# michelbarbeau/gr-uwspr

Hardware: NVIDIA B200
Metric: WSPR windows/sec (coarse+fine sync+demod) (higher is better)
Workload: dtype f32

## Files before the change

gr-uwspr_b200/csrc/capi.cu:

```cuda
#include <limits.h>
#include <math.h>
#include <stdio.h>
#include <stdlib.h>
#include <string.h>

#include <algorithm>
#include <chrono>
#include <future>
#include <string>
#include <thread>
#include <vector>

#include "common.cuh"
#include "../host/wspr_tables.h"

#ifndef M_PI
#define M_PI 3.14159265358979323846
#endif

namespace {

const int kMaxChunks = 1024;
const int kCounterSets = 15;
const int kCounterInts = 4 + 4 * kCounterSets;
// ... 1012 lines not shown
        for (int r = 0; r < d.n_rows; r++) memcpy(ps + (size_t)r * d.n_bins, &tmp[(size_t)r * d.nbp], sizeof(float) * d.n_bins);
    }
    if (psavg) CU(cudaMemcpy(psavg, ctx->b.psavg + slot * d.nbp, sizeof(float) * d.n_bins, cudaMemcpyDeviceToHost));
    return UWSPR_B200_OK;
}

int uwspr_b200_last_timing(const uwspr_b200_ctx *ctx, float ms[4])
{
    if (!ctx || !ms) return UWSPR_B200_E_PARAM;
    for (int q = 0; q < 4; q++) ms[q] = ctx->ms[q];
    return UWSPR_B200_OK;
}

int64_t uwspr_b200_launch_count(const uwspr_b200_ctx *ctx) { return ctx ? ctx->launches : 0; }

}
```

gr-uwspr_b200/csrc/common.cuh:

```cuda
#pragma once

#include <cuda_runtime.h>
#include <stdint.h>

#include "uwspr_b200.h"

#define UW_NSYM 162
#define UW_FFT_N 512
#define UW_HOP 128
#define UW_NK0 26
#define UW_NIFR 5
#define UW_NTRAJ 125
#define UW_SPS 256
#define UW_NP 45000
#define UW_MAX_TILE_W 40
#define UW_MAX_UNIQUE 192
#define UW_NQUAD 41

struct UwDims {
    int fl, n_rows, size, m, hpbm, finpb, noiseidx, maxfreqs, maxcand, maxdrift, cf;
    float df, min_snr, floor_val, threshold;
    int bin_lo, n_bins, nbp;
    int n_lin, n_hyp, n_unique;
    int off_min, off_max, tile_w;
// ... 77 lines not shown
                           const float *window, const float2 *twiddle, float *amp, float *ps_dbg,
                           float *psavg, UwPeak *peaks, int *npk, cudaStream_t s);
void uw_launch_worklist(const int *npk, int nwin, int cap, int *base, UwItem *items, int *counters,
                        int *set, cudaStream_t s);
void uw_launch_coarse(const UwDims &d, const float *amp, const UwPeak *peaks, const UwItem *items,
                      const int *total, int cap, const uint32_t *off4, const short *hyp_unique,
                      uwspr_b200_candidate_t *cands, int *ticket, int grid, cudaStream_t s);
struct UwFineWork {
    void *state;
    float4 *pbuf, *pE, *pbest, *tables;
    int *tickets;
    int slice;
};
cudaError_t uw_fine_work_alloc(UwFineWork *w, int slice);
void uw_fine_work_free(UwFineWork *w);
struct UwFineLaunch {
    int grid_points, grid_lags, grid_share;
    bool lag_share;
    bool reuse;
};
int uw_launch_fine(const UwDims &d, const float2 *x, const UwGeom &geom, const UwItem *items, const int *begin,
                   const int *end, int cap, const uwspr_b200_candidate_t *cands, int jig_first, int jig_count,
                   uwspr_b200_refined_t *refined, uwspr_b200_jiggle_t *jig, uint8_t *soft, int slice0,
                   const UwFineWork &w, const UwFineLaunch &l, cudaStream_t s);
int uw_coarse_fine_channels(uwspr_b200_ctx *ctx, const float *samples, int64_t win_stride, int wins_per_chan,
                            int64_t chan_stride, int nchan, int jig_first, int jig_count, int32_t *npk,
                            uwspr_b200_candidate_t *cands, int cap, int32_t *total);
int64_t uw_frontend_stream_launches(const uwspr_b200_frontend_stream *s);
size_t uw_coarse_smem_bytes(const UwDims &d);
int uw_coarse_setup(const UwDims &d);
int uw_fine_setup(int sm_count, bool lag_share, bool reuse, UwFineLaunch *l);
int uw_coarse_blocks_per_sm(const UwDims &d);
// ... 9 lines not shown
```

gr-uwspr_b200/csrc/fine.cu:

```cuda
#include "common.cuh"

#include <algorithm>
#include <cassert>

namespace {

constexpr int kThreads = 256;
constexpr int kWarps = kThreads / 32;
constexpr int kPB = 5;
constexpr int kKC1 = 8;
constexpr int kPitch1 = kKC1 + 2;
constexpr int kNChunk1 = UW_SPS / kKC1;
constexpr int kRows2 = 32;
constexpr int kPass2 = UW_NSYM / kRows2;
constexpr int kSpan2 = 128;
constexpr int kKCR = 32;
constexpr int kRing = kSpan2 + 2 * kKCR;
constexpr int kPitch2 = kRing + 1;
constexpr int kMaxJ = UWSPR_B200_NJIG;
constexpr int kLagPT = 5;
constexpr int kMemo = 24;
constexpr int kTickets = 16;
constexpr size_t kWarpSmem = 2 * 32 * kPitch1 * sizeof(float2) + 2 * 2 * kKC1 * 2 * sizeof(float4);
constexpr int kSlots1 = (kPB * UW_NSYM + 31) / 32;
constexpr int kSlotsRest = (kMaxJ * (UW_NSYM - kPass2 * kRows2) + 31) / 32;

struct FineCand {
    float f1, drift1, sync1;
    int shift1;
    int worth;
    int npt, nev;
    float pt_f0[kPB];
    int pt_lag[kPB];
    float pt_drift[kPB];
    float pt_ss[kPB];
    int ev[kPB];
    int tab[kPB];
    int ntab;
    float tab_f0[kPB], tab_drift[kPB];
    int memo_n;
    float memo_f0[kMemo], memo_drift[kMemo], memo_ss[kMemo];
    int memo_lag[kMemo];
    int nl;
    int e_lag[kMaxJ], e_jig[kMaxJ];
    float e_f0, e_drift;
    int best_have, best_lag, best_col;
    float best_f0, best_drift;
    int e_reuse;
    int xoff;
};

struct FineConst {
// ... 5 lines not shown
struct FineArgs {
    UwDims d;
    FineConst fc;
    const float2 *x;
    UwGeom geom;
    const UwItem *items;
    const uwspr_b200_candidate_t *cands;
    const int *begin_ptr, *end_ptr;
    int cap, slice0, slice_n;
    FineCand *st;
    float4 *pbuf;
    float4 *pE;
    float4 *pbest;
    float4 *tables;
    int *tickets;
    int jig_first, jig_count;
    int reuse;
    uwspr_b200_refined_t *refined;
    uwspr_b200_jiggle_t *jig;
    uint8_t *soft;
};

__device__ __forceinline__ int slice_count(const FineArgs &a)
{
    const int begin = *a.begin_ptr + a.slice0, end = min(*a.end_ptr, a.cap);
    return max(0, min(a.slice_n, end - begin));
}

__device__ __forceinline__ void cp_async_commit() { asm volatile("cp.async.commit_group;\n" ::: "memory"); }
template <int IMM> __device__ __forceinline__ void cp_async8_s(unsigned sdst, const void *gsrc, int bytes)
// ... 18 lines not shown
    double r = __ddiv_rn(__dmul_rn((double)(-sign), num), den);
    r = __ddiv_rn(__dmul_rn(r, (double)cf), 1500.0);
    return (float)r;
}

__device__ __forceinline__ uwspr_b200_candidate_t load_cand(const uwspr_b200_candidate_t *cands, int g)
{
    uwspr_b200_candidate_t cand = cands[g];
    if (cand.m_type != 0) {
        unsigned long long v1 = (unsigned long long)__double_as_longlong(cand.m_nonlinear.V1);
        cand.m_nonlinear.V1 = __longlong_as_double((long long)(v1 & 0xffffffff00000000ull));
    }
    return cand;
}

__device__ __forceinline__ float symbol_freq(const UwDims &d, const uwspr_b200_candidate_t &cand, float f0,
                                             float drift, int i)
{
    if (cand.m_type == 0) {
        const double a = __dmul_rn((double)drift, 0.5);
        const double b = __dsub_rn((double)(float)i, 81.0);
        return (float)__dadd_rn((double)f0, __ddiv_rn(__dmul_rn(a, b), 81.0));
    }
    const float t = d.nonlinear_intended_t ? (float)(i * 111 / 162) : 0.0f;
    return __fadd_rn(f0, slm_frequency_drift(cand.m_nonlinear.V1, cand.m_nonlinear.V2, cand.m_nonlinear.p1,
                                             cand.m_nonlinear.p2, (float)d.cf, t));
}

__device__ __forceinline__ void tone_seed(const FineConst &fc, float fp, int j, float &cd, float &sd)
{
    const double arg = __dmul_rn(fc.twopidt, (double)__fadd_rn(fp, fc.delta[j]));
    double sn, cs;
    sincos(arg, &sn, &cs);
    cd = (float)cs;
    sd = (float)sn;
}

#define UW_MAC2(inp, quad, xv, c, s)                                                             \
// ... 201 lines not shown
    extern __shared__ __align__(16) unsigned char smem_raw[];
    const int lane = threadIdx.x & 31, warp = threadIdx.x >> 5;
    WarpTile xt = reinterpret_cast<WarpTile>(smem_raw + (size_t)warp * kWarpSmem);
    TableTile tt = reinterpret_cast<TableTile>(smem_raw + (size_t)warp * kWarpSmem + 2 * 32 * kPitch1 * sizeof(float2));
    const int n = slice_count(a);
    const int begin = *a.begin_ptr + a.slice0;
    constexpr int kSlots = REST ? kSlotsRest : kSlots1;
    constexpr int s_lo = REST ? kPass2 * kRows2 : 0, s_cnt = REST ? UW_NSYM - kPass2 * kRows2 : UW_NSYM;
    for (;;) {
        int slot = 0;
        if (lane == 0) slot = atomicAdd(a.tickets + tk, 1);
        slot = __shfl_sync(0xffffffffu, slot, 0);
        if (slot >= n * kSlots) break;
        const int cidx = slot / kSlots, local = slot - cidx * kSlots;
        const FineCand &st = a.st[cidx];
        const int np = REST ? (st.worth == 1 ? st.nl : 0) : (lag_share && st.nev > 0 && st.tab[0] < 0) ? 0 : st.nev;
        const int ntask = np * s_cnt;
        if (local * 32 >= ntask) continue;
        const int g = begin + cidx;
        const uwspr_b200_candidate_t cand = load_cand(a.cands, g);
        const float2 *xw = a.x + st.xoff;
        const int task = local * 32 + lane;
        const bool live = task < ntask;
        const int tq = min(task, ntask - 1);
        const int q = tq / s_cnt;
        const int i = s_lo + (tq - q * s_cnt);
        float f0, drift;
        int lag, tab = -1;
        float4 *out;
        if (REST) {
            f0 = st.e_f0;
            drift = st.e_drift;
            lag = st.e_lag[q];
            out = a.pE + ((size_t)cidx * UW_NSYM + i) * kMaxJ + q;
        } else {
            const int pq = st.ev[q];
            f0 = st.pt_f0[pq];
            drift = st.pt_drift[pq];
            lag = st.pt_lag[pq];
            tab = st.tab[q];
            out = a.pbuf + ((size_t)cidx * UW_NSYM + i) * kPB + q;
        }
        if (!REST && __all_sync(0xffffffffu, tab >= 0)) {
            const int tab_a = __shfl_sync(0xffffffffu, tab, 0), tab_b = __shfl_sync(0xffffffffu, tab, 31);
            const float4 *tbase = a.tables + (size_t)cidx * kPB * (UW_SPS * 2);
            r1_task<true>(xt, tt, a.d, a.fc, xw, cand, live, f0, drift, lag, i, tbase + (size_t)tab_a * (UW_SPS * 2),
                          tbase + (size_t)tab_b * (UW_SPS * 2), tab == tab_a ? 0 : 1, out);
        } else {
            r1_task<false>(xt, tt, a.d, a.fc, xw, cand, live, f0, drift, lag, i, nullptr, nullptr, 0, out);
        }
    }
}

static_assert(UW_SPS % kKCR == 0 && kRing % 8 == 0, "chunks and lag offsets (multiples of 8) never straddle the wrap");

template <int IMM> __device__ __forceinline__ float2 lds_f2(unsigned addr)
// ... 329 lines not shown
        if (!RING || nl == kPB)
            lagshare_run<RING, kPB>(wsm, a.x, rp, rb, pe, cd, sd, inp, quad, nz);
        else
            lagshare_run<RING, kPB - 1>(wsm, a.x, rp, rb, pe, cd, sd, inp, quad, nz);
        if (live) {
            float4 *out = a.pbuf + ((size_t)cidx * UW_NSYM + i) * kPB;
#pragma unroll
            for (int e = 0; e < kPB; e++)
                if (e < nev)
                    out[e] = make_float4(tone_mag(uw_lo(inp[e][0]), uw_lo(quad[e][0])), tone_mag(uw_hi(inp[e][0]), uw_hi(quad[e][0])),
                                         tone_mag(uw_lo(inp[e][1]), uw_lo(quad[e][1])), tone_mag(uw_hi(inp[e][1]), uw_hi(quad[e][1])));
        }
    }
}

__device__ __forceinline__ bool const_freq(bool lin, bool intended_t, float drift)
{
    return lin ? (drift == 0.0f) : !intended_t;
}

__device__ __forceinline__ void stage_points(FineCand &st, int np, bool lin, bool intended_t)
{
    int nev = 0;
    for (int q = 0; q < np; q++) {
        int hit = -1;
        for (int m = 0; m < st.memo_n; m++)
            if (__float_as_uint(st.memo_f0[m]) == __float_as_uint(st.pt_f0[q]) && st.memo_lag[m] == st.pt_lag[q] &&
                __float_as_uint(st.memo_drift[m]) == __float_as_uint(st.pt_drift[q])) {
                hit = m;
                break;
            }
        if (hit >= 0)
            st.pt_ss[q] = st.memo_ss[hit];
        else
            st.ev[nev++] = q;
    }
// ... 5 lines not shown
        int t = -1;
        if (const_freq(lin, intended_t, st.pt_drift[q])) {
            for (int u = 0; u < ntab && t < 0; u++)
                if (__float_as_uint(st.tab_f0[u]) == __float_as_uint(st.pt_f0[q]) &&
                    __float_as_uint(st.tab_drift[u]) == __float_as_uint(st.pt_drift[q]))
                    t = u;
            if (t < 0) {
                t = ntab++;
                st.tab_f0[t] = st.pt_f0[q];
                st.tab_drift[t] = st.pt_drift[q];
            }
        }
        st.tab[e] = t;
    }
    st.ntab = ntab;
}

__device__ __forceinline__ void keep_point(FineCand &st, int q)
{
    st.best_col = -1;
    if (q < 0) return;
    for (int e = 0; e < st.nev; e++)
        if (st.ev[e] == q) {
            st.best_col = e;
            st.best_have = 1;
            st.best_f0 = st.pt_f0[q];
            st.best_lag = st.pt_lag[q];
            st.best_drift = st.pt_drift[q];
        }
}
// ... 10 lines not shown
    st.sync1 = syncmax;
    st.shift1 = (best >= 0) ? st.pt_lag[best] : 0;
    st.f1 = (best >= 0) ? st.pt_f0[best] : 0.0f;
    keep_point(st, best);
}

template <int STAGE>
__global__ void __launch_bounds__(256) k_fine_step(FineArgs a)
{
    const int n = slice_count(a);
    const int begin = *a.begin_ptr + a.slice0;
    const int gt = blockIdx.x * blockDim.x + threadIdx.x;
    const int cidx = gt >> 3, sub = gt & 7;
    const unsigned gmask = 0xffu << (threadIdx.x & 24);
    const bool have = cidx < n;
    __shared__ FineCand s_state[256 / 8];
    static_assert(sizeof(FineCand) % 4 == 0, "copied word by word");
    FineCand &gst = a.st[have ? cidx : 0];
    FineCand &st = s_state[threadIdx.x >> 3];
    if (have) {
        const int *src = reinterpret_cast<const int *>(&gst);
        int *dst = reinterpret_cast<int *>(&st);
        for (int k = sub; k < (int)(sizeof(FineCand) / 4); k += 8) dst[k] = STAGE >= 1 ? src[k] : 0;
    }
    __syncwarp(gmask);
    const int g = begin + cidx;
    const float minsync1 = 0.10f;
    const bool skip = have && STAGE >= 4 && st.worth != 1;
    if (STAGE >= 1 && have && !skip && sub < st.nev) {
        const float4 *p = a.pbuf + (size_t)cidx * UW_NSYM * kPB + sub;
        float ss = 0.0f, totp = 0.0f;
        constexpr int kBatch = 9;
        static_assert(UW_NSYM % kBatch == 0, "162 = 18 x 9");
        for (int i0 = 0; i0 < UW_NSYM; i0 += kBatch) {
            float4 vb[kBatch];
#pragma unroll
            for (int k = 0; k < kBatch; k++) vb[k] = p[(size_t)(i0 + k) * kPB];
#pragma unroll
            for (int k = 0; k < kBatch; k++) {
                const float4 v = vb[k];
                totp = __fadd_rn(__fadd_rn(__fadd_rn(__fadd_rn(totp, v.x), v.y), v.z), v.w);
                const float cmet = __fsub_rn(__fadd_rn(v.y, v.w), __fadd_rn(v.x, v.z));
                ss = uw_sync_bit(a.d.sync_words, i0 + k) ? __fadd_rn(ss, cmet) : __fsub_rn(ss, cmet);
// ... 6 lines not shown
    if (sub == 0) {
        const uwspr_b200_candidate_t cand = a.cands[g];
        const bool lin = cand.m_type == 0;
        if (STAGE == 0) {
            st.f1 = cand.freq;
            st.drift1 = lin ? cand.m_linear.drift : 0.0f;
            st.shift1 = cand.shift;
            st.sync1 = cand.sync;
            st.memo_n = 0;
            st.worth = -1;
            st.nl = 0;
            st.best_have = 0;
            st.best_col = -1;
            st.e_reuse = -1;
            st.xoff = (int)(uw_window_offset(a.geom, a.items[g].win) - uw_window_offset(a.geom, 0));
            if (cidx == 0)
                for (int q = 0; q < kTickets; q++) a.tickets[q] = 0;
        } else {
            for (int e = 0; e < st.nev && st.memo_n < kMemo; e++) {
                const int q = st.ev[e], m = st.memo_n++;
                st.memo_f0[m] = st.pt_f0[q];
                st.memo_lag[m] = st.pt_lag[q];
                st.memo_drift[m] = st.pt_drift[q];
                st.memo_ss[m] = st.pt_ss[q];
            }
        }
        if (STAGE == 1 || STAGE == 2 || STAGE == 4 || STAGE == 5) select_best(st);
        if (STAGE == 3) st.best_col = -1;
        if (STAGE == 3 && lin) {
            const float syncp = (st.pt_ss[0] > -1e30f) ? st.pt_ss[0] : -1e30f;
            const float syncm = (st.pt_ss[1] > -1e30f) ? st.pt_ss[1] : -1e30f;
            if (!(st.pt_ss[1] > -1e30f)) {
// ... 28 lines not shown
            const float fstep = STAGE == 1 ? 0.25f : 0.05f;
            for (int q = 0; q < 5; q++) {
                st.pt_f0[q] = __fadd_rn(f1, __fmul_rn((float)(q - 2), fstep));
                st.pt_lag[q] = shift1;
                st.pt_drift[q] = drift1;
            }
            np = 5;
        } else if (STAGE == 2 && lin) {
            for (int q = 0; q < 2; q++) {
                st.pt_f0[q] = __fadd_rn(f1, __fmul_rn(0.0f, 0.0f));
                st.pt_lag[q] = shift1;
                st.pt_drift[q] = (float)((double)drift1 + (q == 0 ? 0.5 : -0.5));
            }
            np = 2;
        }
        if (STAGE <= 4) stage_points(st, np, lin, a.d.nonlinear_intended_t != 0);
        const bool final_state = (STAGE == 3 && st.worth == 0) || STAGE == 5;
        if (final_state && a.refined) {
            uwspr_b200_refined_t r;
            r.f1 = st.f1;
            r.shift1 = st.shift1;
            r.drift1 = st.drift1;
            r.sync1 = st.sync1;
            r.worth_a_try = st.worth == 1 ? 1 : 0;
            r.reserved = 0;
            a.refined[g] = r;
        }
        if (STAGE == 5) {
            st.e_f0 = __fadd_rn(st.f1, __fmul_rn(0.0f, 0.0f));
            st.e_drift = st.drift1;
            const bool reuse = st.best_have && __float_as_uint(st.best_f0) == __float_as_uint(st.e_f0) &&
// ... 7 lines not shown
                if (idt >= a.jig_first && idt < a.jig_first + a.jig_count && !(reuse && idt == 0)) {
                    st.e_lag[nl] = st.shift1 + off;
                    st.e_jig[nl] = idt - a.jig_first;
                    nl++;
                }
            }
            st.nl = nl;
            st.nev = 0;
        }
    }
    __syncwarp(gmask);
    {
        const int *src = reinterpret_cast<const int *>(&st);
        int *dst = reinterpret_cast<int *>(&gst);
        for (int k = sub; k < (int)(sizeof(FineCand) / 4); k += 8) dst[k] = src[k];
    }
    if (STAGE >= 1 && st.best_col >= 0) {
        const float4 *src = a.pbuf + (size_t)cidx * UW_NSYM * kPB + st.best_col;
        float4 *dst = a.pbest + (size_t)cidx * UW_NSYM;
        for (int i = sub; i < UW_NSYM; i += 8) dst[i] = src[(size_t)i * kPB];
    }
    if (STAGE == 3 && st.worth == 0) {
        uint8_t *soft_g = a.soft ? a.soft + (long long)g * a.jig_count * UW_NSYM : nullptr;
        uwspr_b200_jiggle_t *jig_g = a.jig ? a.jig + (long long)g * a.jig_count : nullptr;
        if (soft_g)
            for (int t = sub; t < a.jig_count * UW_NSYM; t += 8) soft_g[t] = 0;
        if (jig_g)
            for (int t = sub; t < a.jig_count; t += 8) {
                uwspr_b200_jiggle_t z;
                z.sync = 0.0f;
// ... 72 lines not shown
    if (a.jig) {
        uwspr_b200_jiggle_t r;
        const float sy = (sync > -1e30f) ? sync : -1e30f;
        r.sync = sy;
        r.rms = (float)__dsqrt_rn(__ddiv_rn((double)(float)sq, 162.0));
        r.shift = kept ? st.shift1 : st.e_lag[slot];
        r.gate = (sy > minsync2 && r.rms > minrms) ? 1 : 0;
        a.jig[(long long)g * a.jig_count + jidx] = r;
    }
}

constexpr size_t kPointsSmem = (size_t)kWarps * kWarpSmem;

}

cudaError_t uw_fine_work_alloc(UwFineWork *w, int slice)
{
    *w = UwFineWork{};
    const size_t n = (size_t)slice;
    const size_t bytes[6] = { n * sizeof(FineCand), n * UW_NSYM * kPB * sizeof(float4), n * UW_NSYM * kMaxJ * sizeof(float4),
                              n * UW_NSYM * sizeof(float4), n * kPB * UW_SPS * 2 * sizeof(float4), kTickets * sizeof(int) };
    size_t at[7] = { 0 };
    for (int q = 0; q < 6; q++) at[q + 1] = at[q] + ((bytes[q] + 255) & ~(size_t)255);
    char *p = nullptr;
    const cudaError_t e = cudaMalloc(&p, at[6]);
    if (e != cudaSuccess) return e;
    *w = UwFineWork{ p, reinterpret_cast<float4 *>(p + at[1]), reinterpret_cast<float4 *>(p + at[2]),
                     reinterpret_cast<float4 *>(p + at[3]), reinterpret_cast<float4 *>(p + at[4]),
                     reinterpret_cast<int *>(p + at[5]), slice };
    return cudaMemset(w->tickets, 0, kTickets * sizeof(int));
}

void uw_fine_work_free(UwFineWork *w)
{
    if (w->state) cudaFree(w->state);
    *w = UwFineWork{};
}

int uw_fine_setup(int sm_count, bool lag_share, bool reuse, UwFineLaunch *l)
{
    if (cudaFuncSetAttribute(k_fine_lags, cudaFuncAttributeMaxDynamicSharedMemorySize, (int)sizeof(LagSmem)) != cudaSuccess) return 1;
    if (cudaFuncSetAttribute(k_fine_points<false>, cudaFuncAttributeMaxDynamicSharedMemorySize, (int)kPointsSmem) != cudaSuccess) return 1;
    if (cudaFuncSetAttribute(k_fine_points<true>, cudaFuncAttributeMaxDynamicSharedMemorySize, (int)kPointsSmem) != cudaSuccess) return 1;
    if (cudaFuncSetAttribute(k_fine_lagshare<false>, cudaFuncAttributeMaxDynamicSharedMemorySize, (int)kShareSmem) != cudaSuccess) return 1;
    if (cudaFuncSetAttribute(k_fine_lagshare<true>, cudaFuncAttributeMaxDynamicSharedMemorySize, (int)kShareSmem) != cudaSuccess) return 1;
    int n = 0, m = 0;
    const int points = (cudaOccupancyMaxActiveBlocksPerMultiprocessor(&n, k_fine_points<false>, kThreads, kPointsSmem) == cudaSuccess && n > 0) ? n : 1;
    const int lags = (cudaOccupancyMaxActiveBlocksPerMultiprocessor(&n, k_fine_lags, kThreads, sizeof(LagSmem)) == cudaSuccess && n > 0) ? n : 1;
    const bool ok = cudaOccupancyMaxActiveBlocksPerMultiprocessor(&n, k_fine_lagshare<false>, kShareThreads, kShareSmem) == cudaSuccess &&
                    cudaOccupancyMaxActiveBlocksPerMultiprocessor(&m, k_fine_lagshare<true>, kShareThreads, kShareSmem) == cudaSuccess;
    const int share = (ok && std::min(n, m) > 0) ? std::min(n, m) : 1;
    *l = UwFineLaunch{ sm_count * points, sm_count * lags, sm_count * share, lag_share, reuse };
    return 0;
}

int uw_launch_fine(const UwDims &d, const float2 *x, const UwGeom &geom, const UwItem *items, const int *begin,
                   const int *end, int cap, const uwspr_b200_candidate_t *cands, int jig_first, int jig_count,
                   uwspr_b200_refined_t *refined, uwspr_b200_jiggle_t *jig, uint8_t *soft, int slice0,
                   const UwFineWork &w, const UwFineLaunch &l, cudaStream_t s)
{
    const int slice_n = w.slice;
    FineArgs a;
    a.reuse = l.reuse ? 1 : 0;
    a.pbest = w.pbest;
    a.tables = w.tables;
    a.tickets = w.tickets;
    a.d = d;
// ... 9 lines not shown
    a.items = items;
    a.cands = cands;
    a.begin_ptr = begin;
    a.end_ptr = end;
    a.cap = cap;
    a.slice0 = slice0;
    a.slice_n = slice_n;
    a.st = static_cast<FineCand *>(w.state);
    a.pbuf = w.pbuf;
    a.pE = w.pE;
    a.jig_first = jig_first;
    a.jig_count = jig_count;
    a.refined = refined;
    a.jig = jig;
    a.soft = soft;
    const int step_grid = (slice_n * 8 + 255) / 256;
    int launches = 0;
#define UW_STEP(S)                                         \
    k_fine_step<S><<<step_grid, 256, 0, s>>>(a);          \
    launches++
    int tk = 0;
    const bool share = l.lag_share;
#define UW_POINTS(LAGS)                                                                     \
    k_fine_tables<<<(slice_n * 32 + 127) / 128, 128, 0, s>>>(a);                           \
    k_fine_points<false><<<l.grid_points, kThreads, kPointsSmem, s>>>(a, tk++, LAGS && share); \
    launches += 2
    UW_STEP(0);
    UW_POINTS(1);
    if (share) {
        k_fine_lagshare<false><<<l.grid_share, kShareThreads, kShareSmem, s>>>(a, tk++);
        launches++;
    }
    UW_STEP(1);
    UW_POINTS(0);
    UW_STEP(2);
    UW_POINTS(0);
    UW_STEP(3);
    UW_POINTS(1);
    if (share) {
        k_fine_lagshare<true><<<l.grid_share, kShareThreads, kShareSmem, s>>>(a, tk++);
        launches++;
    }
    UW_STEP(4);
    UW_POINTS(0);
    UW_STEP(5);
#undef UW_STEP
#undef UW_POINTS
    if (jig_count > 0) {
        k_fine_lags<<<l.grid_lags, kThreads, sizeof(LagSmem), s>>>(a, tk++);
        k_fine_points<true><<<l.grid_points, kThreads, kPointsSmem, s>>>(a, tk++, 0);
        k_fine_finish<<<(slice_n * 32 + 127) / 128, 128, 0, s>>>(a);
        launches += 3;
    }
    assert(tk <= kTickets);
    return launches;
}
```

gr-uwspr_b200/uwspr_b200/binding.py:

```python
import ctypes as C
import os

import numpy as np

_HERE = os.path.dirname(os.path.abspath(__file__))
NSYM = 162
NJIG = 17
HOST, DEVICE = 0, 1

EXPORTED_SYMBOLS = [
    "uwspr_b200_create", "uwspr_b200_destroy", "uwspr_b200_last_error", "uwspr_b200_status_string",
    "uwspr_b200_create_error", "uwspr_b200_info", "uwspr_b200_coarse", "uwspr_b200_fine", "uwspr_b200_coarse_fine",
    "uwspr_b200_deinterleave", "uwspr_b200_fano", "uwspr_b200_decode_candidate", "uwspr_b200_decode_batch",
    "uwspr_b200_host_alloc",
    "uwspr_b200_host_free", "uwspr_b200_set_stream", "uwspr_b200_set_debug", "uwspr_b200_debug_spectrogram",
    "uwspr_b200_last_timing", "uwspr_b200_launch_count",
    "uwspr_b200_receiver_create", "uwspr_b200_receiver_destroy", "uwspr_b200_receiver_push", "uwspr_b200_receiver_pop",
    "uwspr_b200_receiver_windows", "uwspr_b200_hashtab_bytes", "uwspr_b200_unpack", "uwspr_b200_format_message_log",
    "uwspr_b200_pack_type1", "uwspr_b200_channel_symbols", "uwspr_b200_read_c2", "uwspr_b200_frontend", "uwspr_b200_frontend_ctaps",
    "uwspr_b200_frontend_error", "uwspr_b200_coarse_fine_submit", "uwspr_b200_poll", "uwspr_b200_wait",
    "uwspr_b200_decode_device", "uwspr_b200_fano_batch",
    "uwspr_b200_frontend_stream_create", "uwspr_b200_frontend_stream_push", "uwspr_b200_frontend_stream_outputs",
    "uwspr_b200_frontend_stream_destroy", "uwspr_b200_array_receiver_create", "uwspr_b200_array_receiver_push",
    "uwspr_b200_array_receiver_pop", "uwspr_b200_array_receiver_windows", "uwspr_b200_array_receiver_launch_count",
    "uwspr_b200_array_receiver_destroy",
]

CAND_DTYPE = np.dtype(
    {
        "names": ["freq", "snr", "drift", "sync", "shift", "m_type", "lin_drift", "V1", "V2", "p1", "p2"],
        "formats": ["<f4", "<f4", "<f4", "<f4", "<i4", "<i4", "<f4", "<f8", "<f8", "<i4", "<i4"],
# ... 94 lines not shown
    L.uwspr_b200_frontend_ctaps.argtypes = L.uwspr_b200_frontend.argtypes
    L.uwspr_b200_frontend_error.restype = C.c_char_p
    L.uwspr_b200_host_alloc.restype = C.c_int
    L.uwspr_b200_host_alloc.argtypes = [C.POINTER(vp), C.c_size_t]
    L.uwspr_b200_host_free.argtypes = [vp]
    L.uwspr_b200_set_stream.restype = C.c_int
    L.uwspr_b200_set_stream.argtypes = [vp, vp]
    L.uwspr_b200_set_debug.restype = C.c_int
    L.uwspr_b200_set_debug.argtypes = [vp, C.c_int]
    L.uwspr_b200_debug_spectrogram.restype = C.c_int
    L.uwspr_b200_debug_spectrogram.argtypes = [vp, C.c_int, vp, vp]
    L.uwspr_b200_last_timing.restype = C.c_int
    L.uwspr_b200_last_timing.argtypes = [vp, vp]
    L.uwspr_b200_launch_count.restype = i64
    L.uwspr_b200_launch_count.argtypes = [vp]
    L.uwspr_b200_receiver_create.restype = C.c_int
    L.uwspr_b200_receiver_create.argtypes = [C.POINTER(Params), C.c_int, C.c_int, C.POINTER(vp)]
    L.uwspr_b200_receiver_destroy.argtypes = [vp]
    L.uwspr_b200_receiver_push.restype = C.c_int
    L.uwspr_b200_receiver_push.argtypes = [vp, vp, i64, C.c_int]
    L.uwspr_b200_receiver_pop.restype = C.c_int
    L.uwspr_b200_receiver_pop.argtypes = [vp, vp, vp, vp]
    L.uwspr_b200_receiver_windows.restype = i64
    L.uwspr_b200_receiver_windows.argtypes = [vp]
    L.uwspr_b200_frontend_stream_create.restype = C.c_int
    L.uwspr_b200_frontend_stream_create.argtypes = [C.c_int, C.c_int, C.c_int, vp, C.c_int, C.c_int, C.c_int, C.c_int, C.c_double,
                                                    C.c_double, C.POINTER(vp)]
    L.uwspr_b200_frontend_stream_push.restype = C.c_int
    L.uwspr_b200_frontend_stream_push.argtypes = [vp, vp, C.c_int, i64, i64, vp, C.c_int, i64, i64, C.POINTER(i64)]
    L.uwspr_b200_frontend_stream_outputs.restype = i64
# ... 221 lines not shown

    def debug_spectrogram(self, win=0):
        ps = np.zeros((self.info.n_rows, self.info.n_bins), np.float32)
        psavg = np.zeros(self.info.n_bins, np.float32)
        self._check(self.L.uwspr_b200_debug_spectrogram(self.h, win, _p(ps), _p(psavg)))
        return ps, psavg

    def last_timing(self):
        ms = (C.c_float * 4)()
        self._check(self.L.uwspr_b200_last_timing(self.h, ms))
        return [float(v) for v in ms]

    def launch_count(self):
        return int(self.L.uwspr_b200_launch_count(self.h))


def deinterleave(sym):
    s = np.array(sym, dtype=np.uint8, copy=True)
    load_library().uwspr_b200_deinterleave(_p(s))
    return s


def fano(symbols, delta=60, maxcycles=10000, nbits=81):
    s = np.ascontiguousarray(symbols, dtype=np.uint8)
    data = np.zeros(11, np.uint8)
    metric, cycles, maxnp = C.c_uint32(), C.c_uint32(), C.c_uint32()
    r = load_library().uwspr_b200_fano(C.byref(metric), C.byref(cycles), C.byref(maxnp), _p(data), _p(s), nbits, delta, maxcycles)
    return r, data, metric.value, cycles.value, maxnp.value


# ... 369 lines not shown
```

include/uwspr_b200.h:

```cpp
#ifndef UWSPR_B200_H
#define UWSPR_B200_H

#include <stddef.h>
#include <stdint.h>

#ifdef __cplusplus
extern "C" {
#endif

#define UWSPR_B200_API __attribute__((visibility("default")))

enum {
    UWSPR_B200_OK = 0,
    UWSPR_B200_E_PARAM = 1,
    UWSPR_B200_E_CUDA = 2,
    UWSPR_B200_E_CAPACITY = 3,
    UWSPR_B200_E_NOMEM = 4,
    UWSPR_B200_E_STATE = 5
};

enum { UWSPR_B200_HOST = 0, UWSPR_B200_DEVICE = 1 };

#define UWSPR_B200_NSYM 162
#define UWSPR_B200_NJIG 17
// ... 161 lines not shown
UWSPR_B200_API int64_t uwspr_b200_array_receiver_windows(const uwspr_b200_array_receiver *rx);
UWSPR_B200_API int64_t uwspr_b200_array_receiver_launch_count(const uwspr_b200_array_receiver *rx);
UWSPR_B200_API void uwspr_b200_array_receiver_destroy(uwspr_b200_array_receiver *rx);

UWSPR_B200_API int uwspr_b200_host_alloc(void **ptr, size_t bytes);
UWSPR_B200_API void uwspr_b200_host_free(void *ptr);

UWSPR_B200_API int uwspr_b200_set_stream(uwspr_b200_ctx *ctx, void *cuda_stream);

UWSPR_B200_API int uwspr_b200_set_debug(uwspr_b200_ctx *ctx, int keep_power);

UWSPR_B200_API int uwspr_b200_debug_spectrogram(uwspr_b200_ctx *ctx, int win, float *ps, float *psavg);

UWSPR_B200_API int uwspr_b200_last_timing(const uwspr_b200_ctx *ctx, float ms[4]);
UWSPR_B200_API int64_t uwspr_b200_launch_count(const uwspr_b200_ctx *ctx);

#ifdef __cplusplus
}
#endif
#endif
```

Baseline: 338,700.

## Share fine-sync correlation across candidates with identical frequency trajectories

Adds a hash-based classing step in fine sync: probe points whose (f0, drift) key matches are grouped into classes, and a new class-share kernel computes the tone correlation once per class while feeding several consumers with different lags and offsets. This removes duplicated oscillator and seed work across candidates at stages 1, 2 and 4. In exchange it adds three launches per stage (scan, scatter, class kernel), hash tables and extra workspace, and it can only help when enough points fall into shared classes. It also adds an API for reading the class counts.

```diff
diff --git a/gr-uwspr_b200/csrc/capi.cu b/gr-uwspr_b200/csrc/capi.cu
--- a/gr-uwspr_b200/csrc/capi.cu
+++ b/gr-uwspr_b200/csrc/capi.cu
@@ -1050,4 +1050,16 @@
 
 int64_t uwspr_b200_launch_count(const uwspr_b200_ctx *ctx) { return ctx ? ctx->launches : 0; }
 
-}
+int uwspr_b200_fine_class_counts(uwspr_b200_ctx *ctx, int64_t counts[6])
+{
+    if (!ctx || !counts) return UWSPR_B200_E_PARAM;
+    CU(cudaSetDevice(ctx->device));
+    CU(cudaDeviceSynchronize());
+    long long c[6] = { 0 };
+    for (const UwFineWork &w : ctx->b.fine)
+        if (uw_fine_class_counts(w, c)) return fail(ctx, UWSPR_B200_E_CUDA, "reading the class counts failed");
+    for (int q = 0; q < 6; q++) counts[q] = c[q];
+    return UWSPR_B200_OK;
+}
+
+}
diff --git a/gr-uwspr_b200/csrc/common.cuh b/gr-uwspr_b200/csrc/common.cuh
--- a/gr-uwspr_b200/csrc/common.cuh
+++ b/gr-uwspr_b200/csrc/common.cuh
@@ -115,8 +115,9 @@
 };
 cudaError_t uw_fine_work_alloc(UwFineWork *w, int slice);
 void uw_fine_work_free(UwFineWork *w);
+int uw_fine_class_counts(const UwFineWork &w, long long counts[6]);
 struct UwFineLaunch {
-    int grid_points, grid_lags, grid_share;
+    int grid_points, grid_lags, grid_share, grid_class;
     bool lag_share;
     bool reuse;
 };
diff --git a/gr-uwspr_b200/csrc/fine.cu b/gr-uwspr_b200/csrc/fine.cu
--- a/gr-uwspr_b200/csrc/fine.cu
+++ b/gr-uwspr_b200/csrc/fine.cu
@@ -20,7 +20,12 @@
 constexpr int kMaxJ = UWSPR_B200_NJIG;
 constexpr int kLagPT = 5;
 constexpr int kMemo = 24;
-constexpr int kTickets = 16;
+constexpr int kHeavy = 16;
+constexpr int kClassStages = 3;
+constexpr int kTickets = kHeavy + 2 * kClassStages;
+constexpr int kTotalsAt = 32;
+static_assert(kTickets <= kTotalsAt, "counters and totals do not overlap");
+__host__ __device__ constexpr int class_counter(int stage) { return kHeavy + 2 * (stage == 1 ? 0 : stage == 2 ? 1 : 2); }
 constexpr size_t kWarpSmem = 2 * 32 * kPitch1 * sizeof(float2) + 2 * 2 * kKC1 * 2 * sizeof(float4);
 constexpr int kSlots1 = (kPB * UW_NSYM + 31) / 32;
 constexpr int kSlotsRest = (kMaxJ * (UW_NSYM - kPass2 * kRows2) + 31) / 32;
@@ -36,6 +41,7 @@
     float pt_ss[kPB];
     int ev[kPB];
     int tab[kPB];
+    int n1, ev1[kPB];
     int ntab;
     float tab_f0[kPB], tab_drift[kPB];
     int memo_n;
@@ -71,6 +77,16 @@
     float4 *pbest;
     float4 *tables;
     int *tickets;
+    int class_share;
+    int hbits;
+    unsigned long long *hkey;
+    int *hcnt, *hcls;
+    int *clist;
+    int4 *cinfo;
+    int2 *ptcls;
+    int4 *ctask;
+    int4 *ccons;
+    unsigned long long *totals;
     int jig_first, jig_count;
     int reuse;
     uwspr_b200_refined_t *refined;
@@ -119,14 +135,17 @@
     return cand;
 }
 
+__device__ __forceinline__ float linear_freq(float f0, float drift, int i)
+{
+    const double a = __dmul_rn((double)drift, 0.5);
+    const double b = __dsub_rn((double)(float)i, 81.0);
+    return (float)__dadd_rn((double)f0, __ddiv_rn(__dmul_rn(a, b), 81.0));
+}
+
 __device__ __forceinline__ float symbol_freq(const UwDims &d, const uwspr_b200_candidate_t &cand, float f0,
                                              float drift, int i)
 {
-    if (cand.m_type == 0) {
-        const double a = __dmul_rn((double)drift, 0.5);
-        const double b = __dsub_rn((double)(float)i, 81.0);
-        return (float)__dadd_rn((double)f0, __ddiv_rn(__dmul_rn(a, b), 81.0));
-    }
+    if (cand.m_type == 0) return linear_freq(f0, drift, i);
     const float t = d.nonlinear_intended_t ? (float)(i * 111 / 162) : 0.0f;
     return __fadd_rn(f0, slm_frequency_drift(cand.m_nonlinear.V1, cand.m_nonlinear.V2, cand.m_nonlinear.p1,
                                              cand.m_nonlinear.p2, (float)d.cf, t));
@@ -358,7 +377,7 @@
         if (slot >= n * kSlots) break;
         const int cidx = slot / kSlots, local = slot - cidx * kSlots;
         const FineCand &st = a.st[cidx];
-        const int np = REST ? (st.worth == 1 ? st.nl : 0) : (lag_share && st.nev > 0 && st.tab[0] < 0) ? 0 : st.nev;
+        const int np = REST ? (st.worth == 1 ? st.nl : 0) : (lag_share && st.nev > 0 && st.tab[0] < 0) ? 0 : st.n1;
         const int ntask = np * s_cnt;
         if (local * 32 >= ntask) continue;
         const int g = begin + cidx;
@@ -378,12 +397,12 @@
             lag = st.e_lag[q];
             out = a.pE + ((size_t)cidx * UW_NSYM + i) * kMaxJ + q;
         } else {
-            const int pq = st.ev[q];
+            const int e = st.ev1[q], pq = st.ev[e];
             f0 = st.pt_f0[pq];
             drift = st.pt_drift[pq];
             lag = st.pt_lag[pq];
-            tab = st.tab[q];
-            out = a.pbuf + ((size_t)cidx * UW_NSYM + i) * kPB + q;
+            tab = st.tab[e];
+            out = a.pbuf + ((size_t)cidx * UW_NSYM + i) * kPB + e;
         }
         if (!REST && __all_sync(0xffffffffu, tab >= 0)) {
             const int tab_a = __shfl_sync(0xffffffffu, tab, 0), tab_b = __shfl_sync(0xffffffffu, tab, 31);
@@ -743,12 +762,291 @@
     }
 }
 
+constexpr int kClassL = 5;
+static_assert(kClassL <= kPB, "a thread keeps its consumers in kPB-sized arrays");
+constexpr int kClassWarpSmem = 2 * kClassL * kSegB;
+constexpr size_t kClassSmem = (size_t)kShareWarps * kClassWarpSmem;
+constexpr int kClassCtas = 4;
+
+__device__ __forceinline__ unsigned long long class_key(float f0, float drift)
+{
+    return ((unsigned long long)__float_as_uint(f0) << 32) | __float_as_uint(drift);
+}
+
+__device__ __forceinline__ bool class_point(const FineCand &st, int e, bool cls)
+{
+    if (!cls || e >= st.nev) return false;
+    for (int u = 0; u < st.n1; u++)
+        if (st.ev1[u] == e) return false;
+    return true;
+}
+
+__global__ void __launch_bounds__(1024) k_class_scan(FineArgs a, int cc)
+{
+    __shared__ int s_w[32][2];
+    const int lane = threadIdx.x & 31, warp = threadIdx.x >> 5;
+    if (slice_count(a) == 0) return;
+    const int nclass = a.tickets[cc];
+    int cb = 0, tb = 0;
+    for (int c0 = 0; c0 < nclass; c0 += 1024) {
+        const int c = c0 + threadIdx.x;
+        const int h = c < nclass ? a.clist[c] : 0;
+        const int cnt = c < nclass ? a.hcnt[h] : 0, nt = (cnt + kClassL - 1) / kClassL;
+        int x = cnt, y = nt;
+#pragma unroll
+        for (int o = 1; o < 32; o <<= 1) {
+            const int u = __shfl_up_sync(0xffffffffu, x, o), v = __shfl_up_sync(0xffffffffu, y, o);
+            if (lane >= o) {
+                x += u;
+                y += v;
+            }
+        }
+        if (lane == 31) {
+            s_w[warp][0] = x;
+            s_w[warp][1] = y;
+        }
+        __syncthreads();
+        if (warp == 0) {
+            int u = s_w[lane][0], v = s_w[lane][1];
+#pragma unroll
+            for (int o = 1; o < 32; o <<= 1) {
+                const int p = __shfl_up_sync(0xffffffffu, u, o), q = __shfl_up_sync(0xffffffffu, v, o);
+                if (lane >= o) {
+                    u += p;
+                    v += q;
+                }
+            }
+            s_w[lane][0] = u;
+            s_w[lane][1] = v;
+        }
+        __syncthreads();
+        if (c < nclass) {
+            const int wx = warp ? s_w[warp - 1][0] : 0, wy = warp ? s_w[warp - 1][1] : 0;
+            a.cinfo[c] = make_int4(cb + wx + x - cnt, tb + wy + y - nt, cnt, nt);
+            a.hcls[h] = c;
+        }
+        cb += s_w[31][0];
+        tb += s_w[31][1];
+        __syncthreads();
+    }
+    if (threadIdx.x == 0) {
+        a.tickets[cc + 1] = tb;
+        atomicAdd(a.totals + (cc - kHeavy), (unsigned long long)nclass);
+        atomicAdd(a.totals + (cc - kHeavy) + 1, (unsigned long long)tb);
+    }
+}
+
+__global__ void __launch_bounds__(256) k_class_scatter(FineArgs a)
+{
+    const int n = slice_count(a);
+    const int gt = blockIdx.x * blockDim.x + threadIdx.x;
+    const int cidx = gt / kPB, e = gt - cidx * kPB;
+    if (cidx >= n) return;
+    const FineCand &st = a.st[cidx];
+    if (!class_point(st, e, true)) return;
+    const int2 hr = a.ptcls[gt];
+    const int4 ci = a.cinfo[a.hcls[hr.x]];
+    const int q = st.ev[e];
+    a.ccons[ci.x + hr.y] = make_int4(cidx * UW_NSYM * kPB + e, st.xoff, st.pt_lag[q], 0);
+    if (hr.y < ci.w) {
+        const int sz = ci.z / ci.w, rem = ci.z - sz * ci.w;
+        a.ctask[ci.y + hr.y] = make_int4(__float_as_int(st.pt_f0[q]), __float_as_int(st.pt_drift[q]),
+                                         ci.x + hr.y * sz + min(hr.y, rem), sz + (hr.y < rem ? 1 : 0));
+    }
+}
+
+template <bool REST, bool FAST, int NL>
+__device__ __forceinline__ void classshare_run(unsigned wsm, const float2 *x, const float2 *const (&pa)[kPB],
+                                               const int (&nb)[kPB], const int (&xo)[kPB], uw_f2 (&cd)[2],
+                                               uw_f2 (&sd)[2], uw_f2 (&inp)[kPB][2], uw_f2 (&quad)[kPB][2], const uw_f2 nz)
+{
+    const int lane = threadIdx.x & 31, j = lane % kKS;
+    uw_f2 c[2], s[2], c2[2], s2[2];
+#pragma unroll
+    for (int t = 0; t < 2; t++) {
+        c[t] = uw_pk(1.0f, 1.0f);
+        s[t] = uw_pk(0.0f, 0.0f);
+    }
+    constexpr int kNChunk = UW_SPS / kKS;
+    const unsigned dst0 = wsm + (unsigned)((lane / kKS) * kSegPitch * 8 + j * 8);
+#define UW_CLS_STAGE(BUFOFF, CHUNK)                                                                               \
+    do {                                                                                                          \
+        _Pragma("unroll") for (int p = 0; p < NL; p++)                                                            \
+        _Pragma("unroll") for (int e = 0; e < 8; e++) {                                                           \
+            const unsigned d_ = dst0 + (BUFOFF) + (unsigned)(p * kSegB + 4 * e * kSegPitch * 8);                  \
+            const float2 *src_;                                                                                   \
+            bool ok_ = true;                                                                                      \
+            if (REST) {                                                                                           \
+                const int row_ = 4 * e + lane / kKS;                                                              \
+                const int n_ = __shfl_sync(0xffffffffu, nb[p], row_) + j + (CHUNK) * kKS;                         \
+                const int xo_ = __shfl_sync(0xffffffffu, xo[p], row_);                                            \
+                ok_ = (unsigned)(n_ - 1) < (unsigned)(UW_NP - 1);                           \
+                src_ = ok_ ? x + xo_ + n_ : x;                                                                    \
+            } else if (FAST) {                                                                                    \
+                src_ = pa[p] + (4 * e * UW_SPS + (CHUNK) * kKS);                                                  \
+            } else {                                                                                              \
+                const int n_ = nb[p] + 4 * e * UW_SPS + (CHUNK) * kKS;                                            \
+                ok_ = (unsigned)(n_ - 1) < (unsigned)(UW_NP - 1);                                                 \
+                src_ = ok_ ? pa[p] + (4 * e * UW_SPS + (CHUNK) * kKS) : x;                                        \
+            }                                                                                                     \
+            asm volatile("cp.async.ca.shared.global [%0], [%1], 8, %2;\n" ::"r"(d_), "l"(src_), "r"(ok_ ? 8 : 0)  \
+                         : "memory");                                                                             \
+        }                                                                                                         \
+    } while (0)
+    UW_CLS_STAGE(0u, 0);
+    cp_async_commit();
+#pragma unroll 1
+    for (int k = 0; k < kNChunk; k++) {
+        if (k + 1 < kNChunk) UW_CLS_STAGE((unsigned)(((k + 1) & 1) * kClassL * kSegB), k + 1);
+        cp_async_commit();
+        cp_async_wait<1>();
+        __syncwarp();
+        unsigned ad[NL];
+#pragma unroll
+        for (int l = 0; l < NL; l++) ad[l] = wsm + (unsigned)((k & 1) * kClassL * kSegB + l * kSegB + lane * kSegPitch * 8);
+#pragma unroll 1
+        for (int h = 0; h < kKS / 4; h++) {
+#define UW_CLS_STEP(Q, CN, SN, C, S)                                                     \
+    do {                                                                                 \
+        _Pragma("unroll") for (int l = 0; l < NL; l++) {                                 \
+            const float2 xv = lds_f2<8 * (Q)>(ad[l]);                                    \
+            UW_MAC2(inp[l][0], quad[l][0], xv, C[0], S[0]);                              \
+            UW_MAC2(inp[l][1], quad[l][1], xv, C[1], S[1]);                              \
+        }                                                                                \
+        UW_ROT2_TO(CN[0], SN[0], C[0], S[0], cd[0], sd[0]);                              \
+        UW_ROT2_TO(CN[1], SN[1], C[1], S[1], cd[1], sd[1]);                              \
+    } while (0)
+            UW_CLS_STEP(0, c2, s2, c, s);
+            UW_CLS_STEP(1, c, s, c2, s2);
+            UW_CLS_STEP(2, c2, s2, c, s);
+            UW_CLS_STEP(3, c, s, c2, s2);
+#undef UW_CLS_STEP
+#pragma unroll
+            for (int l = 0; l < NL; l++) ad[l] += 4 * 8;
+        }
+        __syncwarp();
+    }
+    cp_async_wait<0>();
+#undef UW_CLS_STAGE
+}
+
+__global__ void __launch_bounds__(kShareThreads, kClassCtas) k_fine_classshare(FineArgs a, int tk, int cc)
+{
+    extern __shared__ __align__(16) unsigned char smem_raw[];
+    const int lane = threadIdx.x & 31, warp = threadIdx.x >> 5;
+    const unsigned wsm = (unsigned)__cvta_generic_to_shared(smem_raw) + (unsigned)(warp * kClassWarpSmem);
+    if (slice_count(a) == 0) return;
+    const int nclass = a.tickets[cc], ntask = a.tickets[cc + 1];
+    for (int c = blockIdx.x * blockDim.x + threadIdx.x; c < nclass; c += gridDim.x * blockDim.x) {
+        const int h = a.clist[c];
+        a.hkey[h] = ~0ull;
+        a.hcnt[h] = 0;
+    }
+    const int nfull = ntask * kShareFull;
+    const int nslots = nfull + (ntask + kShareRestC - 1) / kShareRestC;
+    const uw_f2 nz = a.fc.nz;
+    for (;;) {
+        int slot = 0;
+        if (lane == 0) slot = atomicAdd(a.tickets + tk, 1);
+        slot = __shfl_sync(0xffffffffu, slot, 0);
+        if (slot >= nslots) break;
+        const bool rest = slot >= nfull;
+        int t, i;
+        if (!rest) {
+            t = slot / kShareFull;
+            i = (slot - t * kShareFull) * 32 + lane;
+        } else {
+            t = (slot - nfull) * kShareRestC + lane / 2;
+            i = kShareFull * 32 + (lane & 1);
+        }
+        const bool live = t < ntask;
+        int nc = 0, ob[kPB], nb[kPB], xo[kPB];
+        uw_f2 cd[2] = { 0ull, 0ull }, sd[2] = { 0ull, 0ull };
+#pragma unroll
+        for (int p = 0; p < kPB; p++) {
+            ob[p] = 0;
+            nb[p] = -(1 << 28);
+            xo[p] = 0;
+        }
+        if (live) {
+            const int4 tq = a.ctask[t];
+            nc = tq.w;
+            const float fp = linear_freq(__int_as_float(tq.x), __int_as_float(tq.y), i);
+#pragma unroll
+            for (int u = 0; u < 2; u++) {
+                float cd0, sd0, cd1, sd1;
+                tone_seed(a.fc, fp, 2 * u, cd0, sd0);
+                tone_seed(a.fc, fp, 2 * u + 1, cd1, sd1);
+                cd[u] = uw_pk(cd0, cd1);
+                sd[u] = uw_pk(sd0, sd1);
+            }
+#pragma unroll
+            for (int p = 0; p < kPB; p++) {
+                const int4 cs = a.ccons[tq.z + min(p, nc - 1)];
+                ob[p] = cs.x + i * kPB;
+                xo[p] = cs.y;
+                nb[p] = cs.z + i * UW_SPS;
+            }
+        }
+        uw_f2 inp[kPB][2], quad[kPB][2];
+#pragma unroll
+        for (int e = 0; e < kPB; e++)
+#pragma unroll
+            for (int u = 0; u < 2; u++) {
+                inp[e][u] = uw_pk(0.0f, 0.0f);
+                quad[e][u] = uw_pk(0.0f, 0.0f);
+            }
+        const int nl = __reduce_max_sync(0xffffffffu, nc);
+        if (rest) {
+            const float2 *pa[kPB] = {};
+            classshare_run<true, false, kClassL>(wsm, a.x, pa, nb, xo, cd, sd, inp, quad, nz);
+        } else {
+            const int dr = (lane / kKS - lane) * UW_SPS + lane % kKS;
+            const float2 *pa[kPB];
+            int sb[kPB];
+            bool in = true;
+#pragma unroll
+            for (int p = 0; p < kPB; p++) {
+                sb[p] = nb[p] + dr;
+                pa[p] = a.x + xo[p] + sb[p];
+                in = in && nb[p] >= 1 && nb[p] + UW_SPS <= UW_NP;
+            }
+            const bool fast = __all_sync(0xffffffffu, in);
+#define UW_CLS_RUN(NL)                                                                      \
+    do {                                                                                    \
+        if (fast)                                                                           \
+            classshare_run<false, true, NL>(wsm, a.x, pa, sb, xo, cd, sd, inp, quad, nz);   \
+        else                                                                                \
+            classshare_run<false, false, NL>(wsm, a.x, pa, sb, xo, cd, sd, inp, quad, nz);  \
+    } while (0)
+            if (nl >= 5 && kClassL >= 5)
+                UW_CLS_RUN(kClassL >= 5 ? 5 : 4);
+            else if (nl == 4)
+                UW_CLS_RUN(4);
+            else if (nl == 3)
+                UW_CLS_RUN(3);
+            else if (nl == 2)
+                UW_CLS_RUN(2);
+            else
+                UW_CLS_RUN(1);
+#undef UW_CLS_RUN
+        }
+        if (live) {
+#pragma unroll
+            for (int p = 0; p < kPB; p++)
+                if (p < nc)
+                    a.pbuf[ob[p]] = make_float4(tone_mag(uw_lo(inp[p][0]), uw_lo(quad[p][0])), tone_mag(uw_hi(inp[p][0]), uw_hi(quad[p][0])),
+                                                tone_mag(uw_lo(inp[p][1]), uw_lo(quad[p][1])), tone_mag(uw_hi(inp[p][1]), uw_hi(quad[p][1])));
+        }
+    }
+}
+
 __device__ __forceinline__ bool const_freq(bool lin, bool intended_t, float drift)
 {
     return lin ? (drift == 0.0f) : !intended_t;
 }
 
-__device__ __forceinline__ void stage_points(FineCand &st, int np, bool lin, bool intended_t)
+__device__ __forceinline__ void stage_points(FineCand &st, int np, bool lin, bool intended_t, bool cls)
 {
     int nev = 0;
     for (int q = 0; q < np; q++) {
@@ -784,6 +1082,12 @@
         st.tab[e] = t;
     }
     st.ntab = ntab;
+    int n1 = 0;
+    for (int e = 0; e < nev; e++) {
+        const int q = st.ev[e];
+        if (!(cls && lin && st.tab[e] < 0 && class_key(st.pt_f0[q], st.pt_drift[q]) != ~0ull)) st.ev1[n1++] = e;
+    }
+    st.n1 = n1;
 }
 
 __device__ __forceinline__ void keep_point(FineCand &st, int q)
@@ -824,6 +1128,8 @@
     const int cidx = gt >> 3, sub = gt & 7;
     const unsigned gmask = 0xffu << (threadIdx.x & 24);
     const bool have = cidx < n;
+    if (STAGE == 0 && gt == 0)
+        for (int q = 0; q < kTickets; q++) a.tickets[q] = 0;
     __shared__ FineCand s_state[256 / 8];
     static_assert(sizeof(FineCand) % 4 == 0, "copied word by word");
     FineCand &gst = a.st[have ? cidx : 0];
@@ -837,6 +1143,7 @@
     const int g = begin + cidx;
     const float minsync1 = 0.10f;
     const bool skip = have && STAGE >= 4 && st.worth != 1;
+    constexpr bool kClassStage = STAGE == 1 || STAGE == 2 || STAGE == 4;
     if (STAGE >= 1 && have && !skip && sub < st.nev) {
         const float4 *p = a.pbuf + (size_t)cidx * UW_NSYM * kPB + sub;
         float ss = 0.0f, totp = 0.0f;
@@ -873,8 +1180,6 @@
             st.best_col = -1;
             st.e_reuse = -1;
             st.xoff = (int)(uw_window_offset(a.geom, a.items[g].win) - uw_window_offset(a.geom, 0));
-            if (cidx == 0)
-                for (int q = 0; q < kTickets; q++) a.tickets[q] = 0;
         } else {
             for (int e = 0; e < st.nev && st.memo_n < kMemo; e++) {
                 const int q = st.ev[e], m = st.memo_n++;
@@ -933,7 +1238,7 @@
             }
             np = 2;
         }
-        if (STAGE <= 4) stage_points(st, np, lin, a.d.nonlinear_intended_t != 0);
+        if (STAGE <= 4) stage_points(st, np, lin, a.d.nonlinear_intended_t != 0, kClassStage && a.class_share);
         const bool final_state = (STAGE == 3 && st.worth == 0) || STAGE == 5;
         if (final_state && a.refined) {
             uwspr_b200_refined_t r;
@@ -971,6 +1276,22 @@
         const int *src = reinterpret_cast<const int *>(&st);
         int *dst = reinterpret_cast<int *>(&gst);
         for (int k = sub; k < (int)(sizeof(FineCand) / 4); k += 8) dst[k] = src[k];
+    }
+    if (kClassStage && a.class_share && class_point(st, sub, true)) {
+        const int q = st.ev[sub];
+        const unsigned long long key = class_key(st.pt_f0[q], st.pt_drift[q]);
+        const unsigned mask = (1u << a.hbits) - 1u;
+        unsigned h = (unsigned)((key * 0x9e3779b97f4a7c15ull) >> (64 - a.hbits));
+        for (;;) {
+            const unsigned long long prev = atomicCAS(a.hkey + h, ~0ull, key);
+            if (prev == ~0ull) {
+                a.clist[atomicAdd(a.tickets + class_counter(STAGE), 1)] = (int)h;
+                break;
+            }
+            if (prev == key) break;
+            h = (h + 1u) & mask;
+        }
+        a.ptcls[(size_t)cidx * kPB + sub] = make_int2((int)h, atomicAdd(a.hcnt + h, 1));
     }
     if (STAGE >= 1 && st.best_col >= 0) {
         const float4 *src = a.pbuf + (size_t)cidx * UW_NSYM * kPB + st.best_col;
@@ -1073,21 +1394,50 @@
 
 }
 
+static int class_hash_bits(int slice)
+{
+    int b = 6;
+    while ((1ll << b) < 2ll * slice * kPB) b++;
+    return b;
+}
+
+static void work_layout(int slice, size_t (&at)[15])
+{
+    const size_t n = (size_t)slice, np = n * kPB, nh = (size_t)1 << class_hash_bits(slice);
+    const size_t bytes[14] = { n * sizeof(FineCand), n * UW_NSYM * kPB * sizeof(float4), n * UW_NSYM * kMaxJ * sizeof(float4),
+                               n * UW_NSYM * sizeof(float4), n * kPB * UW_SPS * 2 * sizeof(float4),
+                               kTotalsAt * sizeof(int) + 2 * kClassStages * sizeof(unsigned long long), nh * sizeof(unsigned long long), nh * sizeof(int), nh * sizeof(int), np * sizeof(int),
+                               np * sizeof(int4), np * sizeof(int2), np * sizeof(int4), np * sizeof(int4) };
+    at[0] = 0;
+    for (int q = 0; q < 14; q++) at[q + 1] = at[q] + ((bytes[q] + 255) & ~(size_t)255);
+}
+
 cudaError_t uw_fine_work_alloc(UwFineWork *w, int slice)
 {
     *w = UwFineWork{};
-    const size_t n = (size_t)slice;
-    const size_t bytes[6] = { n * sizeof(FineCand), n * UW_NSYM * kPB * sizeof(float4), n * UW_NSYM * kMaxJ * sizeof(float4),
-                              n * UW_NSYM * sizeof(float4), n * kPB * UW_SPS * 2 * sizeof(float4), kTickets * sizeof(int) };
-    size_t at[7] = { 0 };
-    for (int q = 0; q < 6; q++) at[q + 1] = at[q] + ((bytes[q] + 255) & ~(size_t)255);
+    size_t at[15];
+    work_layout(slice, at);
     char *p = nullptr;
-    const cudaError_t e = cudaMalloc(&p, at[6]);
+    const cudaError_t e = cudaMalloc(&p, at[14]);
     if (e != cudaSuccess) return e;
     *w = UwFineWork{ p, reinterpret_cast<float4 *>(p + at[1]), reinterpret_cast<float4 *>(p + at[2]),
                      reinterpret_cast<float4 *>(p + at[3]), reinterpret_cast<float4 *>(p + at[4]),
                      reinterpret_cast<int *>(p + at[5]), slice };
-    return cudaMemset(w->tickets, 0, kTickets * sizeof(int));
+    cudaError_t r = cudaMemset(p + at[6], 0xff, at[7] - at[6]);
+    if (r == cudaSuccess) r = cudaMemset(p + at[7], 0, at[8] - at[7]);
+    if (r == cudaSuccess) r = cudaMemset(w->tickets, 0, at[6] - at[5]);
+    return r;
+}
+
+int uw_fine_class_counts(const UwFineWork &w, long long counts[6])
+{
+    unsigned long long v[2 * kClassStages] = {};
+    unsigned long long *dv = reinterpret_cast<unsigned long long *>(w.tickets + kTotalsAt);
+    if (w.tickets && (cudaMemcpy(v, dv, sizeof(v), cudaMemcpyDeviceToHost) != cudaSuccess ||
+                      cudaMemset(dv, 0, sizeof(v)) != cudaSuccess))
+        return 1;
+    for (int q = 0; q < 2 * kClassStages; q++) counts[q] += (long long)v[q];
+    return 0;
 }
 
 void uw_fine_work_free(UwFineWork *w)
@@ -1103,13 +1453,15 @@
     if (cudaFuncSetAttribute(k_fine_points<true>, cudaFuncAttributeMaxDynamicSharedMemorySize, (int)kPointsSmem) != cudaSuccess) return 1;
     if (cudaFuncSetAttribute(k_fine_lagshare<false>, cudaFuncAttributeMaxDynamicSharedMemorySize, (int)kShareSmem) != cudaSuccess) return 1;
     if (cudaFuncSetAttribute(k_fine_lagshare<true>, cudaFuncAttributeMaxDynamicSharedMemorySize, (int)kShareSmem) != cudaSuccess) return 1;
+    if (cudaFuncSetAttribute(k_fine_classshare, cudaFuncAttributeMaxDynamicSharedMemorySize, (int)kClassSmem) != cudaSuccess) return 1;
     int n = 0, m = 0;
     const int points = (cudaOccupancyMaxActiveBlocksPerMultiprocessor(&n, k_fine_points<false>, kThreads, kPointsSmem) == cudaSuccess && n > 0) ? n : 1;
     const int lags = (cudaOccupancyMaxActiveBlocksPerMultiprocessor(&n, k_fine_lags, kThreads, sizeof(LagSmem)) == cudaSuccess && n > 0) ? n : 1;
     const bool ok = cudaOccupancyMaxActiveBlocksPerMultiprocessor(&n, k_fine_lagshare<false>, kShareThreads, kShareSmem) == cudaSuccess &&
                     cudaOccupancyMaxActiveBlocksPerMultiprocessor(&m, k_fine_lagshare<true>, kShareThreads, kShareSmem) == cudaSuccess;
     const int share = (ok && std::min(n, m) > 0) ? std::min(n, m) : 1;
-    *l = UwFineLaunch{ sm_count * points, sm_count * lags, sm_count * share, lag_share, reuse };
+    const int cls = (cudaOccupancyMaxActiveBlocksPerMultiprocessor(&n, k_fine_classshare, kShareThreads, kClassSmem) == cudaSuccess && n > 0) ? n : 1;
+    *l = UwFineLaunch{ sm_count * points, sm_count * lags, sm_count * share, sm_count * cls, lag_share, reuse };
     return 0;
 }
 
@@ -1149,6 +1501,22 @@
     a.refined = refined;
     a.jig = jig;
     a.soft = soft;
+    a.class_share = l.lag_share ? 1 : 0;
+    a.hbits = class_hash_bits(slice_n);
+    {
+        size_t at[15];
+        work_layout(slice_n, at);
+        char *p = static_cast<char *>(w.state);
+        a.hkey = reinterpret_cast<unsigned long long *>(p + at[6]);
+        a.hcnt = reinterpret_cast<int *>(p + at[7]);
+        a.hcls = reinterpret_cast<int *>(p + at[8]);
+        a.clist = reinterpret_cast<int *>(p + at[9]);
+        a.cinfo = reinterpret_cast<int4 *>(p + at[10]);
+        a.ptcls = reinterpret_cast<int2 *>(p + at[11]);
+        a.ctask = reinterpret_cast<int4 *>(p + at[12]);
+        a.ccons = reinterpret_cast<int4 *>(p + at[13]);
+        a.totals = reinterpret_cast<unsigned long long *>(w.tickets + kTotalsAt);
+    }
     const int step_grid = (slice_n * 8 + 255) / 256;
     int launches = 0;
 #define UW_STEP(S)                                         \
@@ -1166,10 +1534,19 @@
         k_fine_lagshare<false><<<l.grid_share, kShareThreads, kShareSmem, s>>>(a, tk++);
         launches++;
     }
+#define UW_CLASSES(S)                                                                                   \
+    if (share) {                                                                                        \
+        k_class_scan<<<1, 1024, 0, s>>>(a, class_counter(S));                                           \
+        k_class_scatter<<<(slice_n * kPB + 255) / 256, 256, 0, s>>>(a);                                 \
+        k_fine_classshare<<<l.grid_class, kShareThreads, kClassSmem, s>>>(a, tk++, class_counter(S));   \
+        launches += 3;                                                                                  \
+    }
     UW_STEP(1);
     UW_POINTS(0);
+    UW_CLASSES(1);
     UW_STEP(2);
     UW_POINTS(0);
+    UW_CLASSES(2);
     UW_STEP(3);
     UW_POINTS(1);
     if (share) {
@@ -1178,15 +1555,17 @@
     }
     UW_STEP(4);
     UW_POINTS(0);
+    UW_CLASSES(4);
     UW_STEP(5);
 #undef UW_STEP
 #undef UW_POINTS
+#undef UW_CLASSES
     if (jig_count > 0) {
         k_fine_lags<<<l.grid_lags, kThreads, sizeof(LagSmem), s>>>(a, tk++);
         k_fine_points<true><<<l.grid_points, kThreads, kPointsSmem, s>>>(a, tk++, 0);
         k_fine_finish<<<(slice_n * 32 + 127) / 128, 128, 0, s>>>(a);
         launches += 3;
     }
-    assert(tk <= kTickets);
+    assert(tk <= kHeavy);
     return launches;
 }
diff --git a/gr-uwspr_b200/uwspr_b200/binding.py b/gr-uwspr_b200/uwspr_b200/binding.py
--- a/gr-uwspr_b200/uwspr_b200/binding.py
+++ b/gr-uwspr_b200/uwspr_b200/binding.py
@@ -14,7 +14,7 @@
     "uwspr_b200_deinterleave", "uwspr_b200_fano", "uwspr_b200_decode_candidate", "uwspr_b200_decode_batch",
     "uwspr_b200_host_alloc",
     "uwspr_b200_host_free", "uwspr_b200_set_stream", "uwspr_b200_set_debug", "uwspr_b200_debug_spectrogram",
-    "uwspr_b200_last_timing", "uwspr_b200_launch_count",
+    "uwspr_b200_last_timing", "uwspr_b200_launch_count", "uwspr_b200_fine_class_counts",
     "uwspr_b200_receiver_create", "uwspr_b200_receiver_destroy", "uwspr_b200_receiver_push", "uwspr_b200_receiver_pop",
     "uwspr_b200_receiver_windows", "uwspr_b200_hashtab_bytes", "uwspr_b200_unpack", "uwspr_b200_format_message_log",
     "uwspr_b200_pack_type1", "uwspr_b200_channel_symbols", "uwspr_b200_read_c2", "uwspr_b200_frontend", "uwspr_b200_frontend_ctaps",
@@ -139,6 +139,9 @@
     L.uwspr_b200_last_timing.argtypes = [vp, vp]
     L.uwspr_b200_launch_count.restype = i64
     L.uwspr_b200_launch_count.argtypes = [vp]
+    if hasattr(L, "uwspr_b200_fine_class_counts"):
+        L.uwspr_b200_fine_class_counts.restype = C.c_int
+        L.uwspr_b200_fine_class_counts.argtypes = [vp, vp]
     L.uwspr_b200_receiver_create.restype = C.c_int
     L.uwspr_b200_receiver_create.argtypes = [C.POINTER(Params), C.c_int, C.c_int, C.POINTER(vp)]
     L.uwspr_b200_receiver_destroy.argtypes = [vp]
@@ -390,6 +393,13 @@
     def launch_count(self):
         return int(self.L.uwspr_b200_launch_count(self.h))
 
+    def fine_class_counts(self):
+        if not hasattr(self.L, "uwspr_b200_fine_class_counts"):
+            return None
+        v = (C.c_int64 * 6)()
+        self._check(self.L.uwspr_b200_fine_class_counts(self.h, v))
+        return {st: (int(v[2 * k]), int(v[2 * k + 1])) for k, st in enumerate(("B", "C", "D-freq"))}
+
 
 def deinterleave(sym):
     s = np.array(sym, dtype=np.uint8, copy=True)
diff --git a/include/uwspr_b200.h b/include/uwspr_b200.h
--- a/include/uwspr_b200.h
+++ b/include/uwspr_b200.h
@@ -199,6 +199,7 @@
 
 UWSPR_B200_API int uwspr_b200_last_timing(const uwspr_b200_ctx *ctx, float ms[4]);
 UWSPR_B200_API int64_t uwspr_b200_launch_count(const uwspr_b200_ctx *ctx);
+UWSPR_B200_API int uwspr_b200_fine_class_counts(uwspr_b200_ctx *ctx, int64_t counts[6]);
 
 #ifdef __cplusplus
 }
```

New measurement: 354,800, median of 6. 1.05x the previous value.
